# Fabstir/fabstir-vectordb

Hardware: AMD Instinct MI355X
Metric: k-NN queries/sec at recall@10>=0.95, 1Mx384 f32 (higher is better)
Workload: dtype f32

## Files before the change

### fabstir-vectordb_amd/csrc/kernels_allow.h

```cpp
#pragma once
#include "common.h"
#include "kernels_scan.h"
#include "score_rows.h"
#include "wave_ops.h"

namespace fvdb {

constexpr unsigned long long kAllowEmpty = ~0ull;

__device__ __forceinline__ uint32_t allow_hash(uint64_t id) {
  id ^= id >> 33;
  id *= 0xff51afd7ed558ccdULL;
  id ^= id >> 33;
  id *= 0xc4ceb9fe1a85ec53ULL;
  id ^= id >> 33;
  return (uint32_t)id;
}

__global__ __launch_bounds__(256) void allow_set_build_kernel(const uint64_t* __restrict__ ids, uint64_t n,
                                                              unsigned long long* __restrict__ table, uint32_t slot_mask) {
  const uint64_t i = (uint64_t)blockIdx.x * blockDim.x + threadIdx.x;
  if (i >= n) return;
  const unsigned long long id = ids[i];
  if (id == kAllowEmpty) return;
  uint32_t h = allow_hash(id) & slot_mask;
  for (uint32_t probe = 0; probe <= slot_mask; ++probe) {
    const unsigned long long prev = atomicCAS(&table[h], kAllowEmpty, id);
    if (prev == kAllowEmpty || prev == id) return;
    h = (h + 1) & slot_mask;
  }
}

__device__ __forceinline__ bool allow_set_has(const unsigned long long* __restrict__ table, uint32_t slot_mask, unsigned long long id) {
  if (id == kAllowEmpty) return false;
  uint32_t h = allow_hash(id) & slot_mask;
  for (uint32_t probe = 0; probe <= slot_mask; ++probe) {
    const unsigned long long v = table[h];
    if (v == id) return true;
    if (v == kAllowEmpty) return false;
    h = (h + 1) & slot_mask;
  }
  return false;
}

__global__ __launch_bounds__(256) void allow_pool_words_kernel(const uint64_t* __restrict__ pool_ids, const uint64_t* __restrict__ pool_valid,
                                                               uint32_t blocks, const unsigned long long* __restrict__ table,
                                                               uint32_t slot_mask, uint64_t* __restrict__ out_words,
                                                               unsigned long long* __restrict__ out_count) {
  const uint32_t lane = threadIdx.x & 63;
  const uint32_t blk = blockIdx.x * 4 + (threadIdx.x >> 6);
  if (blk >= blocks) return;
  const uint64_t live = pool_valid[blk];
  bool in = false;
  if ((live >> lane) & 1) in = allow_set_has(table, slot_mask, pool_ids[(size_t)blk * 64 + lane]);
  const uint64_t word = __ballot(in);
  if (lane == 0) {
    out_words[blk] = word;
    if (word) atomicAdd(out_count, (unsigned long long)__popcll(word));
  }
}

__global__ __launch_bounds__(256) void allow_graph_mark_kernel(const uint32_t* __restrict__ nodes, uint64_t n_allowed, uint32_t n,
                                                               uint32_t* __restrict__ flags) {
  const uint64_t i = (uint64_t)blockIdx.x * blockDim.x + threadIdx.x;
  if (i >= n_allowed) return;
  const uint32_t node = nodes[i];
  if (node < n) flags[node] = 0u;
}

__global__ __launch_bounds__(256) void allow_graph_count_kernel(uint32_t* __restrict__ flags, const uint32_t* __restrict__ deleted, uint32_t n,
                                                                uint32_t* __restrict__ wg_count) {
  __shared__ uint32_t s_cnt[4];
  const uint32_t i = blockIdx.x * 256 + threadIdx.x;
  bool ok = false;
  if (i < n) {
    const uint32_t f = (flags[i] | deleted[i]) ? 1u : 0u;
    flags[i] = f;
    ok = f == 0u;
  }
  const uint64_t m = __ballot(ok);
  if ((threadIdx.x & 63) == 0) s_cnt[threadIdx.x >> 6] = (uint32_t)__popcll(m);
  __syncthreads();
  if (threadIdx.x == 0) wg_count[blockIdx.x] = s_cnt[0] + s_cnt[1] + s_cnt[2] + s_cnt[3];
}

__global__ __launch_bounds__(256) void allow_graph_write_kernel(const uint32_t* __restrict__ flags, uint32_t n, const uint32_t* __restrict__ wg_offset,
                                                                uint32_t* __restrict__ out_nodes) {
  __shared__ uint32_t s_cnt[4];
  const uint32_t lane = threadIdx.x & 63, wave = threadIdx.x >> 6;
  const uint32_t i = blockIdx.x * 256 + threadIdx.x;
  const bool ok = i < n && flags[i] == 0u;
  const uint64_t m = __ballot(ok);
  if (lane == 0) s_cnt[wave] = (uint32_t)__popcll(m);
  __syncthreads();
  uint32_t base = wg_offset[blockIdx.x];
  for (uint32_t w = 0; w < wave; ++w) base += s_cnt[w];
  if (ok) out_nodes[base + ballot_rank(m, lane)] = i;
}

struct AllowGroup {
  const uint32_t* nodes;
  uint32_t n_nodes, reserved;
};
struct AllowScanArgs {
  const void* rows;
  const float* queries;
  const uint32_t* nodes;
  uint32_t dpad, n_nodes, B, k;
  uint32_t slices, slice_len;
  uint64_t* part;
  const AllowGroup* groups;
  const uint32_t* group;
};

template <int KR, typename RT = float, bool GR = false>
__global__ __launch_bounds__(256) void allow_scan_kernel(const AllowScanArgs a) {
  __shared__ __attribute__((aligned(16))) float s_tile[4][kScoreTileFloats];
  const int lane = threadIdx.x & 63;
  const uint32_t w = threadIdx.x >> 6;
  const uint32_t q = blockIdx.x * 4 + w, s = blockIdx.y;
  if (q >= a.B) return;
  const float* qrow = a.queries + (size_t)q * a.dpad;
  const uint32_t* nodes = a.nodes;
  uint32_t n_nodes = a.n_nodes;
  if constexpr (GR) {
    const AllowGroup g = a.groups[a.group[q]];
    nodes = g.nodes;
    n_nodes = g.n_nodes;
  }
  const uint32_t lo = s * a.slice_len;
  const uint32_t hi = min(n_nodes, lo + a.slice_len);
  WaveTopK<KR> tk;
  tk.init();
  uint32_t th = kInf32, tl = kInf32;
  for (uint32_t e0 = lo; e0 < hi; e0 += 64) {
    const uint32_t cnt = min(64u, hi - e0);
    const uint32_t pos = e0 + (uint32_t)lane;
    const bool have = (uint32_t)lane < cnt;
    const uint32_t node = have ? nodes[pos] : 0u;
    const float d = score_rows_wave((const RT*)a.rows, a.dpad, qrow, node, cnt, s_tile[w], lane);
    offer<KR>(tk, a.k, have ? __float_as_uint(d) : kInf32, pos, th, tl, lane);
  }
  uint64_t* out = a.part + ((size_t)s * a.B + q) * a.k;
#pragma unroll
  for (int rr = 0; rr < KR; ++rr) {
    const uint32_t e = rr * 64 + lane;
    if (e < a.k) out[e] = ((uint64_t)tk.hi[rr] << 32) | tk.lo[rr];
  }
}

template <int KR, bool GR = false>
__global__ __launch_bounds__(256) void allow_merge_kernel(const uint64_t* __restrict__ part, const uint32_t* __restrict__ nodes, uint32_t slices,
                                                          uint32_t B, uint32_t k, uint32_t* __restrict__ out_nodes, float* __restrict__ out_dist,
                                                          uint32_t* __restrict__ out_counts, const AllowGroup* __restrict__ groups,
                                                          const uint32_t* __restrict__ group) {
  const int lane = threadIdx.x & 63;
  const uint32_t q = blockIdx.x * 4 + (threadIdx.x >> 6);
  if (q >= B) return;
  if constexpr (GR) nodes = groups[group[q]].nodes;
  WaveTopK<KR> tk;
  tk.init();
  uint32_t th = kInf32, tl = kInf32;
  for (uint32_t s = 0; s < slices; ++s)
    for (uint32_t e0 = 0; e0 < k; e0 += 64) {
      const uint32_t e = e0 + lane;
      uint32_t chi = kInf32, clo = 0;
      if (e < k) {
        const uint64_t key = part[((size_t)s * B + q) * k + e];
        chi = (uint32_t)(key >> 32);
        clo = (uint32_t)key;
      }
      offer<KR>(tk, k, chi, clo, th, tl, lane);
    }
  uint32_t count = 0;
#pragma unroll
  for (int rr = 0; rr < KR; ++rr) {
    const uint32_t e = rr * 64 + lane;
    const bool have = e < k && tk.hi[rr] != kInf32;
    count += __popcll(__ballot(have));
    if (e < k) {
      out_nodes[(size_t)q * k + e] = have ? nodes[tk.lo[rr]] : 0xFFFFFFFFu;
      out_dist[(size_t)q * k + e] = have ? __uint_as_float(tk.hi[rr]) : __uint_as_float(0x7F800000u);
    }
  }
  if (lane == 0) out_counts[q] = count;
}

}
```

### fabstir-vectordb_amd/csrc/kernels_coarse.h

```cpp
#pragma once
#include "common.h"
#include "kernels_scan.h"
#include "score_rows.h"

#pragma clang fp contract(off)

namespace fvdb {

typedef float f32x16v __attribute__((ext_vector_type(16)));

__global__ void row_sqnorm_kernel(const float* __restrict__ x, uint32_t stride, uint32_t d, uint32_t n,
                                  float* __restrict__ norms) {
  const uint32_t i = blockIdx.x * blockDim.x + threadIdx.x;
  if (i >= n) return;
  const float* r = x + (size_t)i * stride;
  float s = 0.0f;
  for (uint32_t j = 0; j < d; ++j) s += r[j] * r[j];
  norms[i] = s;
}

__global__ __launch_bounds__(256) void row_sqnorm_wave_kernel(const float* __restrict__ x, uint32_t stride, uint32_t d,
                                                              uint32_t n, float* __restrict__ norms) {
  const int lane = threadIdx.x & 63;
  const uint32_t i = blockIdx.x * 4 + (threadIdx.x >> 6);
  if (i >= n) return;
  const float* r = x + (size_t)i * stride;
  float s = 0.0f;
  for (uint32_t j = lane; j < d; j += 64) s = __builtin_fmaf(r[j], r[j], s);
#pragma unroll
  for (int o = 32; o > 0; o >>= 1) s += __shfl_xor(s, o);
  if (lane == 0) norms[i] = s;
}

__global__ void max_f32_kernel(const float* __restrict__ v, uint32_t n, float* __restrict__ out) {
  if (blockIdx.x == 0 && threadIdx.x == 0) {
    float m = 0.0f;
    for (uint32_t i = 0; i < n; ++i) m = fmaxf(m, v[i]);
    *out = m;
  }
}

__global__ __launch_bounds__(256) void coarse_gemm_kernel(const float* __restrict__ q, const float* __restrict__ c,
                                                          const float* __restrict__ qn, const float* __restrict__ cn,
                                                          uint32_t B, uint32_t nlist, uint32_t dpad,
                                                          float* __restrict__ A ) {
  const int lane = threadIdx.x & 63;
  const uint32_t wave = blockIdx.x * 4 + (threadIdx.x >> 6);
  const uint32_t tiles_c = (nlist + 63) / 64;
  const uint32_t tb = wave / tiles_c, tc = wave - tb * tiles_c;
  if (tb * 32 >= B) return;
  const uint32_t i = lane & 31, h = lane >> 5;
  const uint32_t qrow = min(tb * 32 + i, B - 1);
  const uint32_t c0row = min(tc * 64 + i, nlist - 1), c1row = min(tc * 64 + 32 + i, nlist - 1);
  const float4* qp = (const float4*)(q + (size_t)qrow * dpad + 8 * h);
  const float4* c0p = (const float4*)(c + (size_t)c0row * dpad + 8 * h);
  const float4* c1p = (const float4*)(c + (size_t)c1row * dpad + 8 * h);
  f32x16v acc0 = {0}, acc1 = {0};
  for (uint32_t k0 = 0; k0 < dpad; k0 += 16) {
    const float4 qa = qp[k0 / 4], qb = qp[k0 / 4 + 1];
    const float4 a0 = c0p[k0 / 4], b0 = c0p[k0 / 4 + 1];
    const float4 a1 = c1p[k0 / 4], b1 = c1p[k0 / 4 + 1];
    const float qv[8] = {qa.x, qa.y, qa.z, qa.w, qb.x, qb.y, qb.z, qb.w};
    const float v0[8] = {a0.x, a0.y, a0.z, a0.w, b0.x, b0.y, b0.z, b0.w};
    const float v1[8] = {a1.x, a1.y, a1.z, a1.w, b1.x, b1.y, b1.z, b1.w};
#pragma unroll
    for (int m = 0; m < 8; ++m) {
      acc0 = __builtin_amdgcn_mfma_f32_32x32x2f32(qv[m], v0[m], acc0, 0, 0, 0);
      acc1 = __builtin_amdgcn_mfma_f32_32x32x2f32(qv[m], v1[m], acc1, 0, 0, 0);
    }
  }
  const uint32_t col0 = tc * 64 + i, col1 = col0 + 32;
  const float cn0 = col0 < nlist ? cn[col0] : 0.0f, cn1 = col1 < nlist ? cn[col1] : 0.0f;
#pragma unroll
  for (int r = 0; r < 16; ++r) {
    const uint32_t row = tb * 32 + (r & 3) + 8 * (r >> 2) + 4 * h;
    if (row < B) {
      const float qq = qn[row];
      if (col0 < nlist) A[(size_t)row * nlist + col0] = fmaxf(qq + cn0 - 2.0f * acc0[r], 0.0f);
      if (col1 < nlist) A[(size_t)row * nlist + col1] = fmaxf(qq + cn1 - 2.0f * acc1[r], 0.0f);
    }
  }
}

__device__ __forceinline__ float exact_centroid_dist(const float* __restrict__ q, const float* __restrict__ crow,
                                                     uint32_t dpad) {
  float acc = 0.0f;
  for (uint32_t j = 0; j < dpad; j += 4) {
    const float4 qv = *(const float4*)(q + j), cv = *(const float4*)(crow + j);
    float t;
    t = qv.x - cv.x; acc = acc + t * t;
    t = qv.y - cv.y; acc = acc + t * t;
    t = qv.z - cv.z; acc = acc + t * t;
    t = qv.w - cv.w; acc = acc + t * t;
  }
  return sqrtf(acc);
}

constexpr int kCoarseRegs = 16;

__global__ __launch_bounds__(256) void coarse_select_kernel(const float* __restrict__ A, const float* __restrict__ q,
                                                            const float* __restrict__ c ,
                                                            const float* __restrict__ qn,
                                                            const float* __restrict__ cn_max, uint32_t B,
                                                            uint32_t nlist, uint32_t d, uint32_t dpad, uint32_t C,
                                                            uint32_t kc, uint32_t* __restrict__ out_probes,
                                                            float* __restrict__ out_dist,
                                                            uint32_t* __restrict__ n_exact_fallbacks) {
  __shared__ __attribute__((aligned(16))) float s_tile[4][kScoreTileFloats];
  const int lane = threadIdx.x & 63;
  const uint32_t b = __builtin_amdgcn_readfirstlane(blockIdx.x * 4 + (threadIdx.x >> 6));
  if (b >= B) return;
  const float* arow = A + (size_t)b * nlist;
  const float* qrow = q + (size_t)b * dpad;
  WaveTopK<1> prop;
  prop.init();
  uint32_t th = kInf32, tl = kInf32;
  if (nlist <= 64u * kCoarseRegs && C <= 64 && C >= 1) {
    __shared__ uint32_t s_sel[4][128];
    uint32_t* sel = s_sel[threadIdx.x >> 6];
    uint32_t v[kCoarseRegs];
    uint32_t lo = kInf32, hi = 0;
#pragma unroll
    for (int r = 0; r < kCoarseRegs; ++r) {
      const uint32_t cc = (uint32_t)r * 64u + (uint32_t)lane;
      v[r] = cc < nlist ? __float_as_uint(arow[cc]) : kInf32;
      lo = min(lo, v[r]);
      if (cc < nlist) hi = max(hi, v[r]);
    }
#pragma unroll
    for (int o = 32; o > 0; o >>= 1) {
      lo = min(lo, (uint32_t)__shfl_xor(lo, o));
      hi = max(hi, (uint32_t)__shfl_xor(hi, o));
    }
    auto count_le = [&](uint32_t t) {
      uint32_t cn = 0;
#pragma unroll
      for (int r = 0; r < kCoarseRegs; ++r) cn += __popcll(__ballot(v[r] <= t));
      return cn;
    };
    const uint32_t want = min(C, nlist);
    uint32_t a = lo, b = hi;
    while (a < b) {
      const uint32_t mid = a + ((b - a) >> 1);
      if (count_le(mid) >= want) b = mid;
      else a = mid + 1;
    }
    const uint32_t t = a;
    uint32_t n_lt = 0;
#pragma unroll
    for (int r = 0; r < kCoarseRegs; ++r) n_lt += __popcll(__ballot(v[r] < t));
    uint32_t w_lt = 0, w_eq = n_lt;
#pragma unroll
    for (int r = 0; r < kCoarseRegs; ++r) {
      const uint32_t cc = (uint32_t)r * 64u + (uint32_t)lane;
      const uint64_t ml = __ballot(v[r] < t), me = __ballot(v[r] == t && cc < nlist);
      const uint64_t below = (1ull << lane) - 1ull;
      if (v[r] < t) {
        const uint32_t sl = w_lt + __popcll(ml & below);
        sel[2 * sl] = v[r];
        sel[2 * sl + 1] = cc;
      } else if (v[r] == t && cc < nlist) {
        const uint32_t sl = w_eq + __popcll(me & below);
        if (sl < want) {
          sel[2 * sl] = v[r];
          sel[2 * sl + 1] = cc;
        }
      }
      w_lt += __popcll(ml);
      w_eq += __popcll(me);
    }
    __builtin_amdgcn_fence(__ATOMIC_ACQ_REL, "wavefront");
    __builtin_amdgcn_wave_barrier();
    uint32_t shi = kInf32, slo = kInf32;
    if ((uint32_t)lane < want) {
      shi = sel[2 * lane];
      slo = sel[2 * lane + 1];
    }
    wave_sort64(shi, slo, lane);
    prop.hi[0] = shi;
    prop.lo[0] = slo;
    prop.kth(C, th, tl);
  } else
  for (uint32_t c0 = 0; c0 < nlist; c0 += 64) {
    const uint32_t cc = c0 + lane;
    uint32_t chi = kInf32, clo = cc;
    if (cc < nlist) chi = __float_as_uint(arow[cc]);
    if (c0 == 0) {
      uint32_t shi = chi, slo = cc < nlist ? cc : kInf32;
      wave_sort64(shi, slo, lane);
      prop.hi[0] = shi;
      prop.lo[0] = slo;
      prop.kth(C, th, tl);
    } else {
      offer<1>(prop, C, chi, clo, th, tl, lane);
    }
  }
  const bool all_in = C >= nlist;
  uint32_t ehi = kInf32, elo = kInf32;
  const bool cand = (uint32_t)lane < C && prop.hi[0] != kInf32;
  const uint32_t ncand = __popcll(__ballot(cand));
  const float dex = score_rows_wave(c, dpad, qrow, cand ? prop.lo[0] : 0u, ncand, s_tile[threadIdx.x >> 6], lane);
  if (cand) {
    ehi = __float_as_uint(dex);
    elo = prop.lo[0];
  }
  wave_sort64(ehi, elo, lane);
  bool proven = all_in;
  if (!all_in) {
    const float a_c = __uint_as_float(th);
    const float nq = sqrtf(qn[b]), ncm = sqrtf(cn_max[0]);
    const float eps = 1.01f * (float)(d + 4) * 5.9604645e-8f * (nq + ncm) * (nq + ncm);
    const float lower = sqrtf(fmaxf(a_c - 2.0f * eps, 0.0f)) * (1.0f - 4.8e-7f);
    const uint32_t kk = min(kc, C);
    const float d_k = __uint_as_float(rlane(ehi, kk - 1));
    proven = rlane(ehi, kk - 1) != kInf32 && d_k < lower;
  }
  if (!proven) {
    WaveTopK<1> ex;
    ex.init();
    uint32_t xh = kInf32, xl = kInf32;
    for (uint32_t c0 = 0; c0 < nlist; c0 += 64) {
      const uint32_t cc = c0 + lane;
      uint32_t chi = kInf32;
      if (cc < nlist) chi = __float_as_uint(exact_centroid_dist(qrow, c + (size_t)cc * dpad, dpad));
      if (c0 == 0) {
        uint32_t shi = chi, slo = cc < nlist ? cc : kInf32;
        wave_sort64(shi, slo, lane);
        ex.hi[0] = shi;
        ex.lo[0] = slo;
        ex.kth(kc, xh, xl);
      } else {
        offer<1>(ex, kc, chi, cc, xh, xl, lane);
      }
    }
    ehi = ex.hi[0];
    elo = ex.lo[0];
    if (lane == 0 && n_exact_fallbacks) atomicAdd(n_exact_fallbacks, 1u);
  }
  if ((uint32_t)lane < kc) {
    const bool have = ehi != kInf32;
    out_probes[(size_t)b * kc + lane] = have ? elo : kInf32;
    if (out_dist) out_dist[(size_t)b * kc + lane] = have ? __uint_as_float(ehi) : __uint_as_float(0x7F800000u);
  }
}

}
```

### fabstir-vectordb_amd/csrc/kernels_mfma.h

```cpp
#pragma once
#include "score_rows.h"
#include "common.h"
#include "kernels_scan.h"

#pragma clang fp contract(off)

#ifndef FVDB_MFMA_WAVES
#define FVDB_MFMA_WAVES 2
#endif

namespace fvdb {

typedef _Float16 h8v __attribute__((ext_vector_type(8)));
typedef __fp16 fp16x2v __attribute__((ext_vector_type(2)));
typedef uint32_t u32x4v __attribute__((ext_vector_type(4)));
__device__ __forceinline__ uint32_t pk_rtz(float a, float b) {
  return __builtin_bit_cast(uint32_t, __builtin_amdgcn_cvt_pkrtz(a, b));
}
typedef float f32x16m __attribute__((ext_vector_type(16)));

constexpr float kHalfMax = 65504.0f;

__global__ void pool_row_norms_kernel(const float* __restrict__ src, uint32_t d, uint64_t n, int f16,
                                      const uint32_t* __restrict__ dst_slot, float* __restrict__ norms,
// ... 389 lines not shown
__device__ __forceinline__ float exact_row_dist(const void* __restrict__ pool_data, uint32_t d4, uint32_t blk, int rl,
                                                const float* __restrict__ q) {
  float acc = 0.0f;
  uint32_t c = 0;
  for (; c + 4 <= d4; c += 4) {
    float x[16];
    load_rows16<ST>(pool_data, blk, d4, c, rl, x);
    const f32x16 qv = cload16(q + 4 * c);
    float t;
#pragma unroll
    for (int i = 0; i < 16; ++i) {
      t = x[i] - qv[i];
      acc = acc + t * t;
    }
  }
  if (ST == 0) {
    const float4* xp = (const float4*)pool_data + (size_t)blk * d4 * 64 + rl;
    for (; c < d4; ++c) {
      const float4 xv = xp[(size_t)c * 64];
      const f32x4 qv = cload((const f32x4*)(q + 4 * c));
      float t;
      t = xv.x - qv.x; acc = acc + t * t;
      t = xv.y - qv.y; acc = acc + t * t;
      t = xv.z - qv.z; acc = acc + t * t;
      t = xv.w - qv.w; acc = acc + t * t;
    }
  }
  return sqrtf(acc);
}

__device__ __forceinline__ float exact_row_dist_rm(const float* __restrict__ x, uint32_t d4, const float* __restrict__ q) {
  float acc = 0.0f;
  const float4* xp = (const float4*)x;
  for (uint32_t c = 0; c < d4; ++c) {
    const float4 xv = xp[c];
    const f32x4 qv = cload((const f32x4*)(q + 4 * c));
    float t;
    t = xv.x - qv.x; acc = acc + t * t;
    t = xv.y - qv.y; acc = acc + t * t;
    t = xv.z - qv.z; acc = acc + t * t;
    t = xv.w - qv.w; acc = acc + t * t;
  }
  return sqrtf(acc);
}

__device__ __forceinline__ float mfma_error_bound(float xmax2, float qn2, float d, int x_rounded) {
  const float xm = sqrtf(xmax2) * 1.000001f, nq = sqrtf(qn2) * 1.000001f;
  if (!(xm < kHalfMax && nq < kHalfMax)) return __builtin_huge_valf();
  const float u10 = 9.765625e-4f, u11 = 4.8828125e-4f, u14 = 6.103515625e-5f, u24 = 5.9604645e-8f;
  const float ux = x_rounded == 0 ? 0.0f : (x_rounded == 1 ? u11 : u10);
  const float rnd = ux + u11 + ux * u11;
  const float e1 = 2.0f * rnd * xm * nq;
  const float e2 = 2.0f * (2.0f * d * u24) * xm * nq;
  const float e3 = 1.01f * (2.0f * d + 16.0f) * u24 * (xm + nq) * (xm + nq);
  const float e4 = 2.0f * u14 * sqrtf(d) * (xm + nq);
  return 1.05f * (e1 + e2 + e3 + e4) + 1e-6f * (xm + nq) * (xm + nq);
}

__global__ __launch_bounds__(256) void threshold_kernel(const uint32_t* __restrict__ slots, const uint32_t* __restrict__ first,
                                                        const float* __restrict__ qn,
                                                        const uint32_t* __restrict__ xmax_bits, uint32_t B, uint32_t ka,
                                                        uint32_t d, int rows_f16, float* __restrict__ thr_out) {
  const int lane = threadIdx.x & 63;
  const uint32_t q = rfl(blockIdx.x * 4 + (threadIdx.x >> 6));
  if (q >= B) return;
  const float inf = __builtin_huge_valf();
  float out = inf;
  if (first[q] != kInf32) {
    uint32_t hi = slots[(size_t)q * 64 + lane], lo = (uint32_t)lane;
    wave_sort64(hi, lo, lane);
    const uint32_t kth = rlane(hi, ka - 1);
    const float E = mfma_error_bound(__uint_as_float(*xmax_bits), qn[q], (float)d, rows_f16);
    if (kth != kInf32 && kth != 0u && E < inf) {
      const float a = funmap_u32(kth);
      out = a + 2.0f * E + 1e-6f * fabsf(a);
    }
  }
  if (lane == 0) thr_out[q] = out;
}

struct ThresholdArgs {
  const void* rows;
  const uint64_t* pool_valid;
  const float* pool_norms;
  uint32_t d4;
  ListTable lists;
  const uint32_t* list_len;
  const uint32_t* probes;
  const _Float16* qh;
  const float* queries;
  const float* qn;
  const uint32_t* xmax_bits;
  uint32_t B, np, ka, dpad, capA, min_rows;
  int rows_f16;
  float* thr;
  const uint32_t* glob_blocks;
};

template <bool HALF>
__global__ __launch_bounds__(256) void threshold_direct_kernel(const ThresholdArgs a) {
  const int lane = threadIdx.x & 63;
  const uint32_t q = rfl(blockIdx.x * 4 + (threadIdx.x >> 6));
  if (q >= a.B) return;
  const float inf = __builtin_huge_valf();
  uint32_t best_l = kInf32, best_len = 0;
  for (uint32_t r0 = 0; r0 < a.np && best_len < a.min_rows; r0 += 64) {
    const uint32_t r = r0 + lane;
    uint32_t L = kInf32, len = 0;
    if (r < a.np) {
      L = a.probes[(size_t)q * a.np + r];
      len = L != kInf32 ? (a.glob_blocks ? a.glob_blocks[L] * 64u : a.list_len[L]) : 0u;
    }
    const uint64_t big = __ballot(len >= a.min_rows);
    if (big) {
      const uint32_t l0 = (uint32_t)__builtin_ctzll(big);
      best_l = rlane(L, l0);
      best_len = rlane(len, l0);
      break;
    }
    uint32_t ml = len, mi = (uint32_t)lane;
#pragma unroll
    for (int o = 32; o > 0; o >>= 1) {
      const uint32_t ol = __shfl_xor(ml, o), oi = __shfl_xor(mi, o);
      if (ol > ml || (ol == ml && oi < mi)) {
        ml = ol;
        mi = oi;
      }
    }
    ml = rfl(ml);
    if (ml > best_len) {
      best_len = ml;
      best_l = rlane(L, rfl(mi));
    }
  }
  float out = inf;
  if (best_l != kInf32 && best_len > 0) {
    const uint32_t b_begin = cload(a.lists.off + best_l);
    const uint32_t nblk = min(cload(a.lists.off + best_l + 1) - b_begin, a.capA);
    float best = inf;
    bool bad = false;
    const uint32_t n8 = a.dpad >> 3;
    for (uint32_t b = 0; b < nblk; ++b) {
      const uint32_t blk = cload(a.lists.blocks + b_begin + b);
      float dot = 0.0f;
      if (HALF) {
        const h8v* xp = (const h8v*)a.rows + (size_t)blk * n8 * 64 + lane;
        const _Float16* qrow = a.qh + (size_t)q * a.dpad;
#pragma unroll 4
        for (uint32_t c = 0; c < n8; ++c) {
          const h8v x = xp[(size_t)c * 64];
          const h8v qv = cload((const h8v*)(qrow + 8 * c));
          typedef _Float16 h2v __attribute__((ext_vector_type(2)));
#pragma unroll
          for (int t = 0; t < 4; ++t)
            dot = __builtin_amdgcn_fdot2(h2v{x[2 * t], x[2 * t + 1]}, h2v{qv[2 * t], qv[2 * t + 1]}, dot, false);
        }
      } else {
        const float4* xp = (const float4*)a.rows + (size_t)blk * a.d4 * 64 + lane;
        const float* qrow = a.queries + (size_t)q * a.dpad;
        for (uint32_t c = 0; c < a.d4; ++c) {
          const float4 x = xp[(size_t)c * 64];
          const f32x4 qv = cload((const f32x4*)(qrow + 4 * c));
          dot = __builtin_fmaf(x.x, qv[0], dot);
          dot = __builtin_fmaf(x.y, qv[1], dot);
          dot = __builtin_fmaf(x.z, qv[2], dot);
          dot = __builtin_fmaf(x.w, qv[3], dot);
        }
      }
      const bool live = (cload(a.pool_valid + blk) >> lane) & 1ull;
      const float v = __builtin_fmaf(-2.0f, dot, a.pool_norms[(size_t)blk * 64 + lane]);
      if (live) {
        if (v != v) bad = true;
        else if (v < best) best = v;
      }
    }
    if (!__ballot(bad)) {
      uint32_t hi = best < inf ? fmap_u32(best) : kInf32, lo = (uint32_t)lane;
      wave_sort64(hi, lo, lane);
      const uint32_t kth = rlane(hi, a.ka - 1);
      const float E = mfma_error_bound(__uint_as_float(*a.xmax_bits), a.qn[q], (float)a.dpad, a.rows_f16);
      if (kth != kInf32 && kth != 0u && E < inf) {
        const float av = funmap_u32(kth);
        out = av + (a.glob_blocks ? 1.0f : 2.0f) * E + 1e-6f * fabsf(av);
      }
    }
  }
  if (lane == 0) a.thr[q] = out;
}

__global__ void thr_combine_kernel(const float* __restrict__ u_all, uint32_t W, uint32_t n, const float* __restrict__ qn,
                                   const uint32_t* __restrict__ xmax_bits, float d, int rows_f16, float* __restrict__ thr) {
  const uint32_t i = blockIdx.x * blockDim.x + threadIdx.x;
  if (i >= n) return;
  float m = __builtin_huge_valf();
  for (uint32_t w = 0; w < W; ++w) m = fminf(m, u_all[(size_t)w * n + i]);
  thr[i] = m + mfma_error_bound(__uint_as_float(*xmax_bits), qn[i], d, rows_f16);
}
#ifdef FVDB_DEV_TOOLS
__global__ __launch_bounds__(1024) void thr_loopback_fill_kernel(float* __restrict__ thr, const float* __restrict__ qn, uint32_t n) {
  __shared__ float s_sum[1024];
  __shared__ uint32_t s_cnt[1024];
  float sum = 0.0f;
  uint32_t cnt = 0;
  for (uint32_t i = threadIdx.x; i < n; i += 1024) {
    const float t = thr[i];
    if (t < __builtin_huge_valf()) {
      sum += t + qn[i];
      cnt += 1;
    }
  }
  s_sum[threadIdx.x] = sum;
  s_cnt[threadIdx.x] = cnt;
  __syncthreads();
  for (uint32_t o = 512; o > 0; o >>= 1) {
    if (threadIdx.x < o) {
      s_sum[threadIdx.x] += s_sum[threadIdx.x + o];
      s_cnt[threadIdx.x] += s_cnt[threadIdx.x + o];
    }
    __syncthreads();
  }
  if (s_cnt[0] == 0) return;
  const float typ = s_sum[0] / (float)s_cnt[0];
  for (uint32_t i = threadIdx.x; i < n; i += 1024)
    if (!(thr[i] < __builtin_huge_valf())) thr[i] = typ - qn[i];
}
#endif

__global__ __launch_bounds__(256) void refine_threshold_kernel(const float* __restrict__ sval, uint32_t* __restrict__ scnt,
                                                               const uint32_t* __restrict__ probes, const float* __restrict__ qn,
                                                               const uint32_t* __restrict__ xmax_bits, uint32_t B, uint32_t np,
                                                               uint32_t ka, uint32_t cmax, uint32_t d, int rows_f16,
                                                               float* __restrict__ thr, uint32_t* __restrict__ probes2,
                                                               uint32_t* __restrict__ n_refined) {
  const int lane = threadIdx.x & 63;
  const uint32_t q = rfl(blockIdx.x * 4 + (threadIdx.x >> 6));
  if (q >= B) return;
  const float inf = __builtin_huge_valf();
  bool again = false;
  if (scnt[q] > cmax) {
    WaveTopK<1> ta;
    ta.init();
    uint32_t th = kInf32, tl = kInf32;
    for (uint32_t s0 = 0; s0 < cmax; s0 += 64) {
      const uint32_t s = s0 + lane;
      uint32_t chi = fmap_u32(sval[(size_t)q * cmax + s]), clo = s;
      if (s0 == 0) {
        wave_sort64(chi, clo, lane);
        ta.hi[0] = chi;
        ta.lo[0] = clo;
        ta.kth(ka, th, tl);
      } else {
        offer<1>(ta, ka, chi, clo, th, tl, lane);
      }
    }
    const float E = mfma_error_bound(__uint_as_float(*xmax_bits), qn[q], (float)d, rows_f16);
    if (th != kInf32 && th != 0u && E < inf) {
      const float a = funmap_u32(th);
      const float t2 = a + 2.0f * E + 1e-6f * fabsf(a);
      if (t2 < thr[q]) {
        again = true;
        if (lane == 0) {
          thr[q] = t2;
          scnt[q] = 0;
          if (n_refined) atomicAdd(n_refined, 1u);
        }
      }
    }
  }
  for (uint32_t r = lane; r < np; r += 64) probes2[(size_t)q * np + r] = again ? probes[(size_t)q * np + r] : kInf32;
}

struct VerifyArgs {
  PoolView pool;
  ListTable lists;
  const uint32_t* probes;
  const uint32_t* glob_blocks;
  const float* queries;
  const float* qn;
  const uint32_t* xmax_bits;
  const float* thr;
  const u32x2* surv;
  const float* sval;
  const uint32_t* scnt;
  uint32_t B, k, ka, nprobe, d, dpad, cmax;
  int rows_f16;
  const float* rows_rm;
  int remote_thr;
  uint64_t* out_ids;
  float* out_dist;
  uint32_t* out_counts;
  uint64_t* out_keys;
  uint32_t* fallbacks;
  uint32_t* reasons;
  uint32_t* fail_list;
  uint32_t* nfail;
};

constexpr uint32_t kSelCand = 256;

template <int ST>
__global__ __launch_bounds__(256) void select_kernel(const VerifyArgs m) {
  __shared__ uint32_t s_base[4][256];
  __shared__ uint32_t s_cand[4][kSelCand];
  __shared__ __attribute__((aligned(16))) float s_tile[4][kScoreTileFloats];
  const int lane = threadIdx.x & 63, w = threadIdx.x >> 6;
  const uint32_t q = rfl(blockIdx.x * 4 + w);
  if (q >= m.B) return;
  const uint32_t np = m.nprobe;
  const float inf = __builtin_huge_valf();
  uint32_t carry = 0;
  for (uint32_t r0 = 0; r0 < np; r0 += 64) {
    const uint32_t r = r0 + lane;
    uint32_t v = 0;
    if (r < np) {
      const uint32_t L = m.probes[(size_t)q * np + r];
      v = L != kInf32 ? m.glob_blocks[L] * 64u : 0u;
    }
    const uint32_t inc = wave_incl_scan_u(v, lane);
    if (r < np) s_base[w][r] = carry + inc - v;
    carry += rlane(inc, 63);
  }

  const uint32_t cnt = m.scnt[q];
  const float E = mfma_error_bound(__uint_as_float(*m.xmax_bits), m.qn[q], (float)m.d, m.rows_f16);
  bool proven = cnt <= m.cmax;
  uint32_t ath = kInf32;
  if (proven && cnt > 0) {
    WaveTopK<1> ta;
    ta.init();
    uint32_t th = kInf32, tl = kInf32;
    for (uint32_t s0 = 0; s0 < cnt; s0 += 64) {
      const uint32_t s = s0 + lane;
      uint32_t chi = kInf32, clo = s;
      if (s < cnt) chi = fmap_u32(m.sval[(size_t)q * m.cmax + s]);
      if (s0 == 0) {
        uint32_t slo = s < cnt ? s : kInf32;
        wave_sort64(chi, slo, lane);
        ta.hi[0] = chi;
        ta.lo[0] = slo;
        ta.kth(m.ka, th, tl);
      } else {
        offer<1>(ta, m.ka, chi, clo, th, tl, lane);
      }
    }
    ath = th;
  }
  float cut = inf;
  if (ath != kInf32 && ath != 0u && E < inf) {
    const float a = funmap_u32(ath);
    cut = a + 2.0f * E + 1e-6f * fabsf(a);
    cut = fminf(cut, m.thr[q]);
  }
  uint32_t reason = proven ? 0u : 1u;
  uint32_t ncand = 0;
  if (proven) {
    for (uint32_t s0 = 0; s0 < cnt && ncand <= kSelCand; s0 += 64) {
      const uint32_t s = s0 + lane;
      const bool c = s < cnt && !(m.sval[(size_t)q * m.cmax + s] > cut);
      const uint64_t mask = __ballot(c);
      const uint32_t slot = ncand + ballot_rank(mask, (uint32_t)lane);
      if (c && slot < kSelCand) s_cand[w][slot] = s;
      ncand += __popcll(mask);
    }
    if (ncand > kSelCand) {
      proven = false;
      reason = 2;
    }
  }
  uint32_t khi = kInf32, klo = kInf32;
  if (proven) {
    const float* qrow = m.queries + (size_t)q * m.dpad;
    WaveTopK<1> best;
    best.init();
    uint32_t bh = kInf32, bl = kInf32;
    const uint32_t keep = min(m.k, 64u);
    for (uint32_t c0 = 0; c0 < ncand || c0 == 0; c0 += 64) {
      const uint32_t nset = min(64u, ncand - c0);
      u32x2 sv = {0u, 0u};
      uint32_t blk = 0, chi = kInf32, clo = kInf32;
      if ((uint32_t)lane < nset) {
        sv = m.surv[(size_t)q * m.cmax + s_cand[w][c0 + lane]];
        const uint32_t L = m.probes[(size_t)q * np + sv.x];
        blk = m.lists.blocks[m.lists.off[L] + (sv.y >> 6)];
        clo = s_base[w][sv.x] + sv.y;
      }
      if (nset > 0) {
        if (ST == 0 && m.rows_rm) {
          const float dsel = score_rows_wave(m.rows_rm, m.dpad, qrow, blk * 64u + (sv.y & 63u), nset, s_tile[w], lane);
          if ((uint32_t)lane < nset) chi = __float_as_uint(dsel);
        } else if ((uint32_t)lane < nset) {
          chi = __float_as_uint(exact_row_dist<ST>(m.pool.data, m.pool.d4, blk, (int)(sv.y & 63), qrow));
        }
      }
      if (c0 == 0) {
        wave_sort64(chi, clo, lane);
        best.hi[0] = chi;
        best.lo[0] = clo;
        best.kth(keep, bh, bl);
      } else {
        offer<1>(best, keep, chi, clo, bh, bl, lane);
      }
      if (ncand == 0) break;
    }
    khi = best.hi[0];
    klo = best.lo[0];
    if (cut < inf) {
      const float S = ((cut - E) + m.qn[q]) * 0.999999f;
      const uint32_t dk = rlane(khi, keep - 1);
      proven = dk != kInf32 && S > 0.0f && __uint_as_float(dk) < sqrtf(S);
      if (!proven) reason = 3;
    } else {
      proven = m.remote_thr || m.thr[q] == inf;
      if (!proven) reason = 4;
    }
  }
  if (!proven) {
    if (lane == 0) {
      m.fail_list[atomicAdd(m.nfail, 1u)] = q;
      if (m.fallbacks) atomicAdd(m.fallbacks, 1u);
      if (m.reasons && reason) atomicAdd(m.reasons + (reason - 1), 1u);
    }
    return;
  }
  const bool have = (uint32_t)lane < m.k && khi != kInf32;
  const uint32_t count = __popcll(__ballot(have));
  if ((uint32_t)lane < m.k) {
    uint64_t id = ~0ull;
    if (have) {
      uint32_t r = 0;
      while (r + 1 < np && s_base[w][r + 1] <= klo) ++r;
      const uint32_t L = m.probes[(size_t)q * np + r];
      const uint32_t pos = klo - s_base[w][r];
      const uint32_t blk = m.lists.blocks[m.lists.off[L] + (pos >> 6)];
      id = m.pool.ids[(size_t)blk * 64 + (pos & 63)];
    }
    const size_t o = (size_t)q * m.k + lane;
    if (m.out_ids) m.out_ids[o] = id;
    if (m.out_dist) m.out_dist[o] = have ? __uint_as_float(khi) : __uint_as_float(0x7F800000u);
    if (m.out_keys) m.out_keys[o] = ((uint64_t)khi << 32) | klo;
  }
  if (lane == 0 && m.out_counts) m.out_counts[q] = count;
}

struct FallbackArgs {
  PoolView pool;
  ListTable lists;
  const uint32_t* probes;
  const float* queries;
  const uint32_t* fail_list;
  const uint32_t* nfail;
  uint32_t* head;
  uint32_t k, nprobe, dpad, segb, maxsegs;
  u32x2* part;
};

template <int ST>
__global__ __launch_bounds__(256) void fallback_scan_kernel(const FallbackArgs a) {
  const int lane = threadIdx.x & 63;
  const uint32_t nfail = cload(a.nfail);
  if (nfail == 0) return;
  const uint32_t per_q = a.nprobe * a.maxsegs;
  const uint32_t total = nfail * per_q;
  for (;;) {
    uint32_t item = 0;
    if (lane == 0) item = atomicAdd(a.head, 1u);
    item = rfl(item);
    if (item >= total) return;
    const uint32_t fi = item / per_q, rem = item - fi * per_q;
    const uint32_t r = rem / a.maxsegs, seg = rem - r * a.maxsegs;
    const uint32_t q = cload(a.fail_list + fi);
    const uint32_t L = a.probes[(size_t)q * a.nprobe + r];
    if (L == kInf32) continue;
    const uint32_t bb = a.lists.off[L], nb = a.lists.off[L + 1] - bb;
    const uint32_t b0 = seg * a.segb;
    if (b0 >= nb) continue;
    const uint32_t b1 = min(b0 + a.segb, nb);
    const float* qrow = a.queries + (size_t)q * a.dpad;
    WaveTopK<1> tk;
    tk.init();
    uint32_t th = kInf32, tl = kInf32;
    for (uint32_t b = b0; b < b1; ++b) {
      const uint32_t blk = a.lists.blocks[bb + b];
      const float dist = exact_row_dist<ST>(a.pool.data, a.pool.d4, blk, lane, qrow);
      const bool live = (a.pool.valid[blk] >> lane) & 1ull;
      uint32_t chi = live ? __float_as_uint(dist) : kInf32;
      uint32_t clo = live ? b * 64 + lane : kInf32;
      if (b == b0) {
        wave_sort64(chi, clo, lane);
        tk.hi[0] = chi;
        tk.lo[0] = clo;
        tk.kth(a.k, th, tl);
      } else {
        offer<1>(tk, a.k, chi, clo, th, tl, lane);
      }
    }
    if ((uint32_t)lane < a.k) {
      u32x2 v;
      v.x = tk.hi[0];
      v.y = tk.lo[0];
      a.part[((size_t)(q * a.nprobe + r) * a.maxsegs + seg) * a.k + lane] = v;
    }
  }
}

}
```

### fabstir-vectordb_amd/csrc/row_types.h

```cpp
#pragma once
#include "common.h"

namespace fvdb {

typedef _Float16 half_t;
typedef _Float16 half2_t __attribute__((ext_vector_type(2)));
typedef _Float16 half4_t __attribute__((ext_vector_type(4)));

template <typename RT>
struct RowVec;
template <>
struct RowVec<float> {
  using Pair = float2;
  using Quad = float4;
  static __device__ __forceinline__ Pair zero_pair() { return make_float2(0.0f, 0.0f); }
};
template <>
struct RowVec<half_t> {
  using Pair = half2_t;
  using Quad = half4_t;
  static __device__ __forceinline__ Pair zero_pair() { return Pair{(half_t)0.0f, (half_t)0.0f}; }
};

__device__ __forceinline__ float row_widen(float v) { return v; }
__device__ __forceinline__ float row_widen(half_t v) { return (float)v; }
__device__ __forceinline__ float2 row_widen(float2 v) { return v; }
__device__ __forceinline__ float2 row_widen(half2_t v) { return make_float2((float)v.x, (float)v.y); }
__device__ __forceinline__ float4 row_widen(float4 v) { return v; }
__device__ __forceinline__ float4 row_widen(half4_t v) { return make_float4((float)v.x, (float)v.y, (float)v.z, (float)v.w); }

template <typename RT>
__device__ __forceinline__ float2 row_pair_f32(const RT* row, uint32_t j) {
  return row_widen(*(const typename RowVec<RT>::Pair*)(row + j));
}

}
```

### fabstir-vectordb_amd/csrc/score_rows.h

```cpp
#pragma once
#include "common.h"
#include "row_types.h"

#pragma clang fp contract(off)

namespace fvdb {

#ifndef FVDB_FAST_ADD_UNROLL
#define FVDB_FAST_ADD_UNROLL 16
#endif
constexpr int kScoreAddUnroll = FVDB_FAST_ADD_UNROLL;
constexpr uint32_t kScoreStride = 132;
constexpr uint32_t kScoreTileFloats = 16 * kScoreStride;

#ifdef FVDB_GRAPH_STAMPS
#define SCORE_STAMP_PARAM , unsigned long long* t_acc = nullptr
#define SCORE_STAMP(var) const unsigned long long var = __builtin_amdgcn_s_memtime()
#define SCORE_STAMP_ADD(slot, a, b) \
  do {                              \
    if (t_acc) t_acc[slot] += (b) - (a); \
  } while (0)
#else
#define SCORE_STAMP_PARAM
#define SCORE_STAMP(var)
#define SCORE_STAMP_ADD(slot, a, b)
#endif

template <typename P, int RC, int NB>
__device__ __forceinline__ void score_products(const P (&x)[RC][NB], int c, const float2 q, float* tile, int lane) {
#pragma unroll
  for (int r = 0; r < RC; ++r) {
    const float2 xv = row_widen(x[r][c]);
    const float t0 = q.x - xv.x, t1 = q.y - xv.y;
    *(float2*)(tile + (uint32_t)r * kScoreStride + 2u * (uint32_t)lane) = make_float2(t0 * t0, t1 * t1);
  }
}

template <int RC>
__device__ __forceinline__ uint32_t score_lane_row(int lane) {
  return (uint32_t)lane < (uint32_t)RC ? (uint32_t)lane : (uint32_t)(RC - 1);
}

__device__ __forceinline__ void score_tile_publish() {
  __builtin_amdgcn_fence(__ATOMIC_RELEASE, "wavefront");
  __builtin_amdgcn_wave_barrier();
}
__device__ __forceinline__ float score_add_row(const float* tile, uint32_t lrow, float acc) {
  const float4* p = (const float4*)(tile + lrow * kScoreStride);
#pragma unroll kScoreAddUnroll
  for (int i = 0; i < 32; ++i) {
    const float4 v = p[i];
    acc = acc + v.x;
    acc = acc + v.y;
    acc = acc + v.z;
    acc = acc + v.w;
  }
  return acc;
}
__device__ __forceinline__ void score_tile_retire() {
  __builtin_amdgcn_fence(__ATOMIC_ACQ_REL, "wavefront");
  __builtin_amdgcn_wave_barrier();
}
__device__ __forceinline__ float score_fold(const float* tile, uint32_t lrow, float acc) {
  score_tile_publish();
  acc = score_add_row(tile, lrow, acc);
  score_tile_retire();
  return acc;
}

template <int NB, int RC, bool FULL, int TILES, typename RT>
__device__ __forceinline__ float score_fixed(const RT* __restrict__ rows, uint32_t dpad, const float2 (&q2)[NB], uint32_t pn,
                                             uint32_t cnt, float* stage, uint32_t tile_floats, int lane SCORE_STAMP_PARAM) {
  static_assert(TILES == 1 || TILES == 2, "one or two product tiles");
  SCORE_STAMP(ta);
  using P = typename RowVec<RT>::Pair;
  P x[RC][NB];
  const uint32_t last = cnt - 1;
#pragma unroll
  for (int r = 0; r < RC; ++r) {
    const uint32_t rr = (uint32_t)r < last ? (uint32_t)r : last;
    const uint32_t node = __builtin_amdgcn_readlane(pn, rr);
    const RT* row = rows + (size_t)node * dpad;
#pragma unroll
    for (int c = 0; c < NB; ++c) {
      const uint32_t j = (uint32_t)c * 128u + 2u * (uint32_t)lane;
      if (FULL) x[r][c] = *(const P*)(row + j);
      else x[r][c] = j < dpad ? *(const P*)(row + j) : RowVec<RT>::zero_pair();
    }
  }
  SCORE_STAMP(tb);
  SCORE_STAMP_ADD(8, ta, tb);
  const uint32_t lrow = score_lane_row<RC>(lane);
  score_products(x, 0, q2[0], stage, lane);
  score_tile_publish();
  SCORE_STAMP(tc1);
  SCORE_STAMP_ADD(9, tb, tc1);
  float acc = 0.0f;
#pragma unroll
  for (int c = 0; c < NB; ++c) {
    const float* cur = TILES == 2 ? stage + (uint32_t)(c & 1) * tile_floats : stage;
    if (TILES == 2 && c + 1 < NB) score_products(x, c + 1, q2[c + 1], stage + (uint32_t)((c + 1) & 1) * tile_floats, lane);
    acc = score_add_row(cur, lrow, acc);
    score_tile_retire();
    if (TILES == 1 && c + 1 < NB) {
      score_products(x, c + 1, q2[c + 1], stage, lane);
      score_tile_publish();
    }
  }
  SCORE_STAMP(tc2);
  SCORE_STAMP_ADD(11, tc1, tc2);
  return sqrtf(acc);
}

template <int RC, typename RT>
__device__ __forceinline__ float score_rows_stream(const RT* __restrict__ rows, uint32_t dpad, const float* __restrict__ q, uint32_t pn,
                                                   uint32_t base, uint32_t cnt, float* tile, int lane) {
  const uint32_t nb = (dpad + 127) >> 7;
  using P = typename RowVec<RT>::Pair;
  const RT* rp[RC];
  const uint32_t last = cnt - 1;
#pragma unroll
  for (int r = 0; r < RC; ++r) {
    const uint32_t rr = (uint32_t)r < last ? (uint32_t)r : last;
    rp[r] = rows + (size_t)__builtin_amdgcn_readlane(pn, base + rr) * dpad;
  }
  const uint32_t j0 = 2u * (uint32_t)lane;
  auto load = [&](uint32_t c, P (&x)[RC][1], float2& qv) {
    const uint32_t j = c * 128u + j0;
    const bool in = j < dpad;
    qv = in ? *(const float2*)(q + j) : make_float2(0.0f, 0.0f);
#pragma unroll
    for (int r = 0; r < RC; ++r) x[r][0] = in ? *(const P*)(rp[r] + j) : RowVec<RT>::zero_pair();
  };
  const uint32_t lrow = score_lane_row<RC>(lane);
  float acc = 0.0f;
  auto fold = [&](const P (&x)[RC][1], const float2 qv) {
    score_products(x, 0, qv, tile, lane);
    acc = score_fold(tile, lrow, acc);
  };
  P xa[RC][1], xb[RC][1];
  float2 qa, qb;
  load(0, xa, qa);
  for (uint32_t c = 0; c < nb; c += 2) {
    if (c + 1 < nb) load(c + 1, xb, qb);
    fold(xa, qa);
    if (c + 1 < nb) {
      if (c + 2 < nb) load(c + 2, xa, qa);
      fold(xb, qb);
    }
  }
  return sqrtf(acc);
}

template <typename RT>
__device__ __forceinline__ float score_rows_upto16(const RT* __restrict__ rows, uint32_t dpad, const float* __restrict__ q, uint32_t pn,
                                                   uint32_t base, uint32_t cnt, float* tile, int lane) {
  if (cnt > 8) return score_rows_stream<16>(rows, dpad, q, pn, base, cnt, tile, lane);
  if (cnt > 4) return score_rows_stream<8>(rows, dpad, q, pn, base, cnt, tile, lane);
  return score_rows_stream<4>(rows, dpad, q, pn, base, cnt, tile, lane);
}

template <typename RT>
__device__ __forceinline__ float score_rows_wave(const RT* __restrict__ rows, uint32_t dpad, const float* __restrict__ q, uint32_t pn,
                                                 uint32_t n, float* tile, int lane) {
  float out = 0.0f;
  for (uint32_t base = 0; base < n; base += 16) {
    const uint32_t cnt = min(16u, n - base);
    const float d = score_rows_upto16(rows, dpad, q, pn, base, cnt, tile, lane);
    const float mine = __shfl(d, (int)((uint32_t)lane - base) & 63);
    if ((uint32_t)lane >= base && (uint32_t)lane < base + cnt) out = mine;
  }
  return out;
}

}
```

Before: 1.876 million.

## Score up to 64 rows per wave with quad loads and a wider LDS tile

Adds a score_rows_fold64 path used when a wave scores more than 16 rows. Each lane loads float4 slices so that 8 lanes cover 32 dims of one row, writes the squared differences into a 64-row LDS tile, and then reduces its own row. This replaces the repeated 16-row passes with their shuffles, aiming for wider loads and fewer passes. It also vectorises the pair-product path with ext_vector types and enlarges the shared tile in every kernel that uses it, which raises LDS use and may lower occupancy.

```diff
diff --git a/fabstir-vectordb_amd/csrc/kernels_allow.h b/fabstir-vectordb_amd/csrc/kernels_allow.h
--- a/fabstir-vectordb_amd/csrc/kernels_allow.h
+++ b/fabstir-vectordb_amd/csrc/kernels_allow.h
@@ -115,7 +115,7 @@
 
 template <int KR, typename RT = float, bool GR = false>
 __global__ __launch_bounds__(256) void allow_scan_kernel(const AllowScanArgs a) {
-  __shared__ __attribute__((aligned(16))) float s_tile[4][kScoreTileFloats];
+  __shared__ __attribute__((aligned(16))) float s_tile[4][kScoreTile64Floats];
   const int lane = threadIdx.x & 63;
   const uint32_t w = threadIdx.x >> 6;
   const uint32_t q = blockIdx.x * 4 + w, s = blockIdx.y;
diff --git a/fabstir-vectordb_amd/csrc/kernels_coarse.h b/fabstir-vectordb_amd/csrc/kernels_coarse.h
--- a/fabstir-vectordb_amd/csrc/kernels_coarse.h
+++ b/fabstir-vectordb_amd/csrc/kernels_coarse.h
@@ -106,7 +106,7 @@
                                                             uint32_t kc, uint32_t* __restrict__ out_probes,
                                                             float* __restrict__ out_dist,
                                                             uint32_t* __restrict__ n_exact_fallbacks) {
-  __shared__ __attribute__((aligned(16))) float s_tile[4][kScoreTileFloats];
+  __shared__ __attribute__((aligned(16))) float s_tile[4][kScoreTile64Floats];
   const int lane = threadIdx.x & 63;
   const uint32_t b = __builtin_amdgcn_readfirstlane(blockIdx.x * 4 + (threadIdx.x >> 6));
   if (b >= B) return;
diff --git a/fabstir-vectordb_amd/csrc/kernels_mfma.h b/fabstir-vectordb_amd/csrc/kernels_mfma.h
--- a/fabstir-vectordb_amd/csrc/kernels_mfma.h
+++ b/fabstir-vectordb_amd/csrc/kernels_mfma.h
@@ -715,7 +715,7 @@
 __global__ __launch_bounds__(256) void select_kernel(const VerifyArgs m) {
   __shared__ uint32_t s_base[4][256];
   __shared__ uint32_t s_cand[4][kSelCand];
-  __shared__ __attribute__((aligned(16))) float s_tile[4][kScoreTileFloats];
+  __shared__ __attribute__((aligned(16))) float s_tile[4][kScoreTile64Floats];
   const int lane = threadIdx.x & 63, w = threadIdx.x >> 6;
   const uint32_t q = rfl(blockIdx.x * 4 + w);
   if (q >= m.B) return;
diff --git a/fabstir-vectordb_amd/csrc/row_types.h b/fabstir-vectordb_amd/csrc/row_types.h
--- a/fabstir-vectordb_amd/csrc/row_types.h
+++ b/fabstir-vectordb_amd/csrc/row_types.h
@@ -22,16 +22,22 @@
   static __device__ __forceinline__ Pair zero_pair() { return Pair{(half_t)0.0f, (half_t)0.0f}; }
 };
 
+typedef float f32x2_t __attribute__((ext_vector_type(2)));
+typedef float f32x4_t __attribute__((ext_vector_type(4)));
+__device__ __forceinline__ f32x2_t pack2(float2 v) { return f32x2_t{v.x, v.y}; }
+__device__ __forceinline__ f32x4_t pack4(float4 v) { return f32x4_t{v.x, v.y, v.z, v.w}; }
+
 __device__ __forceinline__ float row_widen(float v) { return v; }
 __device__ __forceinline__ float row_widen(half_t v) { return (float)v; }
-__device__ __forceinline__ float2 row_widen(float2 v) { return v; }
-__device__ __forceinline__ float2 row_widen(half2_t v) { return make_float2((float)v.x, (float)v.y); }
+__device__ __forceinline__ f32x2_t row_widen(float2 v) { return pack2(v); }
+__device__ __forceinline__ f32x2_t row_widen(half2_t v) { return __builtin_convertvector(v, f32x2_t); }
 __device__ __forceinline__ float4 row_widen(float4 v) { return v; }
 __device__ __forceinline__ float4 row_widen(half4_t v) { return make_float4((float)v.x, (float)v.y, (float)v.z, (float)v.w); }
 
 template <typename RT>
 __device__ __forceinline__ float2 row_pair_f32(const RT* row, uint32_t j) {
-  return row_widen(*(const typename RowVec<RT>::Pair*)(row + j));
+  const f32x2_t v = row_widen(*(const typename RowVec<RT>::Pair*)(row + j));
+  return make_float2(v.x, v.y);
 }
 
 }
diff --git a/fabstir-vectordb_amd/csrc/score_rows.h b/fabstir-vectordb_amd/csrc/score_rows.h
--- a/fabstir-vectordb_amd/csrc/score_rows.h
+++ b/fabstir-vectordb_amd/csrc/score_rows.h
@@ -28,11 +28,11 @@
 
 template <typename P, int RC, int NB>
 __device__ __forceinline__ void score_products(const P (&x)[RC][NB], int c, const float2 q, float* tile, int lane) {
+  const f32x2_t qv = pack2(q);
 #pragma unroll
   for (int r = 0; r < RC; ++r) {
-    const float2 xv = row_widen(x[r][c]);
-    const float t0 = q.x - xv.x, t1 = q.y - xv.y;
-    *(float2*)(tile + (uint32_t)r * kScoreStride + 2u * (uint32_t)lane) = make_float2(t0 * t0, t1 * t1);
+    const f32x2_t t = qv - row_widen(x[r][c]);
+    *(f32x2_t*)(tile + (uint32_t)r * kScoreStride + 2u * (uint32_t)lane) = t * t;
   }
 }
 
@@ -160,9 +160,67 @@
   return score_rows_stream<4>(rows, dpad, q, pn, base, cnt, tile, lane);
 }
 
+constexpr uint32_t kScoreStride64 = 36;
+constexpr uint32_t kScoreTile64Floats = 64 * kScoreStride64;
+static_assert(kScoreTile64Floats >= kScoreTileFloats, "one tile for both schedules");
+
+template <typename RT>
+__device__ __forceinline__ float score_rows_fold64(const RT* __restrict__ rows, uint32_t dpad, const float* __restrict__ q, uint32_t pn,
+                                                   uint32_t n, float* tile, int lane) {
+  using Q = typename RowVec<RT>::Quad;
+  const uint32_t sub = 4u * ((uint32_t)lane & 7u), rg = (uint32_t)lane >> 3;
+  const uint32_t ns = (dpad + 31) >> 5, last = n - 1;
+  const RT* rp[8];
+#pragma unroll
+  for (int i = 0; i < 8; ++i) {
+    const uint32_t r = min(8u * (uint32_t)i + rg, last);
+    rp[i] = rows + (size_t)__shfl(pn, (int)r) * dpad + sub;
+  }
+  auto load = [&](uint32_t s, Q (&x)[8], float4& qv) {
+    const uint32_t j = s * 32u;
+    const bool in = j + sub < dpad;
+    qv = in ? *(const float4*)(q + j + sub) : make_float4(0.0f, 0.0f, 0.0f, 0.0f);
+#pragma unroll
+    for (int i = 0; i < 8; ++i) x[i] = in ? *(const Q*)(rp[i] + j) : Q{};
+  };
+  float acc = 0.0f;
+  auto fold = [&](const Q (&x)[8], const float4 qv) {
+    const f32x4_t qq = pack4(qv);
+#pragma unroll
+    for (int i = 0; i < 8; ++i) {
+      const f32x4_t t = qq - pack4(row_widen(x[i]));
+      *(f32x4_t*)(tile + (8u * (uint32_t)i + rg) * kScoreStride64 + sub) = t * t;
+    }
+    score_tile_publish();
+    const float4* p = (const float4*)(tile + (uint32_t)lane * kScoreStride64);
+#pragma unroll
+    for (int i = 0; i < 8; ++i) {
+      const float4 v = p[i];
+      acc = acc + v.x;
+      acc = acc + v.y;
+      acc = acc + v.z;
+      acc = acc + v.w;
+    }
+    score_tile_retire();
+  };
+  Q xa[8], xb[8];
+  float4 qa, qb;
+  load(0, xa, qa);
+  for (uint32_t s = 0; s < ns; s += 2) {
+    if (s + 1 < ns) load(s + 1, xb, qb);
+    fold(xa, qa);
+    if (s + 1 < ns) {
+      if (s + 2 < ns) load(s + 2, xa, qa);
+      fold(xb, qb);
+    }
+  }
+  return sqrtf(acc);
+}
+
 template <typename RT>
 __device__ __forceinline__ float score_rows_wave(const RT* __restrict__ rows, uint32_t dpad, const float* __restrict__ q, uint32_t pn,
                                                  uint32_t n, float* tile, int lane) {
+  if (n > 16) return score_rows_fold64(rows, dpad, q, pn, n, tile, lane);
   float out = 0.0f;
   for (uint32_t base = 0; base < n; base += 16) {
     const uint32_t cnt = min(16u, n - base);
```

Result: no change. 1.881 million (median of 2 runs) (+0.2%).
